# 0xk0ry/HTR-VT

Measured on AMD Instinct MI355X. Metric: line-images/sec (64x1024, global B=128, 128 per GPU) fwd+bwd+CTC, higher is better.
Workload: dtype bf16; 1 GPU; HTR-VT (d768/4L/6h, nb_cls 80) training step: fwd + fused CTC + bwd + AdamW; image=1x64x1024, batch_per_gpu=128, global_batch=128, mask=span 0.4/8 (run/iam.sh), parallelism=dp1, graph_replay=False

## Files before the change

htr-vt_amd/csrc/gemm_halo_impl.h:

```cpp
#pragma once
#include "gemm_dma_impl.h"

namespace {

template <int BN>
struct HaloGeo {
  static constexpr int BM = 256;
  static constexpr int A_PIECES = 40;
  static constexpr int A_STAGE = A_PIECES * 1024;
  static constexpr int B_STAGE = Geo<BN>::BYTES;
  static constexpr int NP_B = B_STAGE / 1024 / 4;
  static constexpr int NP_AH = A_PIECES / 2 / 4;
  static constexpr unsigned B_BASE = 2 * A_STAGE;
  static constexpr int LDS_BYTES = 2 * A_STAGE + 3 * B_STAGE;
  static_assert(B_STAGE % 4096 == 0, "B pieces divide over the four loader waves");
  static_assert(LDS_BYTES <= 160 * 1024, "LDS");
};


typedef float f32x4h_t __attribute__((ext_vector_type(4)));
template <int BN, int TM, int TN>
__device__ __forceinline__ void halo_mma16(f32x4h_t (&a4)[2 * TM][2 * TN], const char* sa, const char* sb, int shift, int wm, int wn,
                                           int lane) {
  const int arow16 = wm * 64 + (lane & 15), ag = lane >> 4;
// ... 40 lines not shown
  const int lr = lane & 15, lg = lane >> 4;
  float s1[2 * TN], s2[2 * TN];
#pragma unroll
  for (int j = 0; j < 2 * TN; ++j) s1[j] = s2[j] = 0.f;
  if (active) {
#pragma unroll
    for (int j = 0; j < 2 * TN; ++j) {
      const int n = n0 + wn * TN * 32 + 16 * j + lr;
      const bool nok = n < p.N;
#pragma unroll
      for (int i = 0; i < 2 * TM; ++i) {
#pragma unroll
        for (int r = 0; r < 4; ++r) {
          const int m = m0 + wm * 64 + 16 * i + 4 * lg + r;
          const float a = a4[i][j][r];
          if constexpr (CSTATS) {
            s1[j] += a;
            s2[j] = fmaf(a, a, s2[j]);
          }
          if (nok && m < p.M) {
            const long long o = (long long)m * p.ldc + n;
            float v = a * p.alpha;
            if (Rf != nullptr) v += Rf[o];
            Cf[o] = v;
          }
        }
      }
    }
  }
  if constexpr (CSTATS) {
    if (p.colstats != nullptr) {
      float* red = reinterpret_cast<float*>(smem);
#pragma unroll
      for (int j = 0; j < 2 * TN; ++j) {
        float a = s1[j], q = s2[j];
        a += __shfl_xor(a, 16, 64); q += __shfl_xor(q, 16, 64);
        a += __shfl_xor(a, 32, 64); q += __shfl_xor(q, 32, 64);
        if (lane < 16 && active) {
          const int c = wn * TN * 32 + 16 * j + lane;
          red[(wm * BN + c) * 2 + 0] = a;
          red[(wm * BN + c) * 2 + 1] = q;
        }
      }
      __syncthreads();
      for (int c = threadIdx.x; c < BN; c += NTH) {
        const int n = n0 + c;
        if (n < p.N) {
          float a = 0.f, q = 0.f;
#pragma unroll
          for (int w = 0; w < 4; ++w) {
            a += red[(w * BN + c) * 2];
            q += red[(w * BN + c) * 2 + 1];
          }
          float* dst = p.colstats + (long long)tile_m * 2 * p.N;
          dst[n] = a;
          dst[p.N + n] = q;
        }
      }
    }
  }
}

template <int BN, class P>
__device__ __forceinline__ void gemm_halo_s2_body(const P& p, const int block_x) {
  using H = HaloGeo<BN>;
  constexpr int BM = 256, NWC = 8, NW_TOTAL = 12, TM = 2, TN = BN / 64;
  extern __shared__ __attribute__((aligned(16))) char smem[];

  const int ntiles = p.tiles_m * p.tiles_n;
  int id = block_x;
  if ((ntiles & 7) == 0) id = (id & 7) * (ntiles >> 3) + (id >> 3);
  const int tile_m = id / p.tiles_n, tile_n = id - tile_m * p.tiles_n;
  const int n0 = tile_n * BN;
  const int sw = p.sw, ncls = 2 * sw;
  const int segs = p.Wq >> 8;
  const int per_row = ncls * segs;
  const int rowq = tile_m / per_row, rem = tile_m - rowq * per_row;
  const int cidx = rem / segs, seg = rem - cidx * segs;
  const int ca = 1 - cidx / sw;
  const int cb = sw == 2 ? 1 - (cidx & 1) : 0;
  const int bimg = rowq / p.Hq, hq = rowq - bimg * p.Hq;
  const int wq0 = seg << 8;
  const int Hh = p.Ho, Ww = p.Wo, Cs = p.Co;
  const int nrow = ca ? 2 : 1;
  const int dyp = ca ? (0 | (2 << 2)) : 1;
  const int dhp = ca ? (1 | (0 << 2)) : 0;
  const int ncol = sw == 1 ? 3 : (cb ? 2 : 1);
  const int dxp = sw == 1 ? (0 | (1 << 2) | (2 << 4)) : (cb ? (0 | (2 << 2)) : 1);
  const int shp = sw == 1 ? (2 | (1 << 2) | (0 << 4)) : (cb ? (2 | (1 << 2)) : 1);
  const int NC = p.Cpad / BK;
  const bool has_x = p.extra_off != 0 && ca == 0 && cb == 0;
  const int nmain = nrow * NC;
  const int ngroups = nmain + (has_x ? NC : 0);
  const int xtap = p.kh * p.kw;
  const int kend = (xtap + 1) * p.Cpad;

  const int lane = threadIdx.x & 63;
  const int wave = __builtin_amdgcn_readfirstlane(threadIdx.x >> 6);
  const bool consumer = wave < NWC;
  const int lw = (wave - NWC) & 3;
  const int wm = (wave >> 1) & 3, wn = wave & 1;
  if (!consumer) __builtin_amdgcn_s_setprio(3);

  DmaLoader<BN, HTRVT_KMAJOR, 0, 4> lb;
  lb.init(p, p.B, p.ldb, n0, p.N, lw, lane);
  const unsigned long long ba = (unsigned long long)p.A;
  const i32x4_t rsrcA = i32x4_t{(int)(unsigned)(ba & 0xffffffffull), (int)(unsigned)((ba >> 32) & 0xffffull), (int)OOB, 0x00020000};
  const int rho0 = lw * 8 + (lane >> 3);
  const int cgA = (lane & 7) ^ Geo<BM>::swz(rho0);
  const unsigned lane_off = (unsigned)((wq0 - 1 + rho0) * Cs + cgA * 8) * 2u;
  const unsigned lds0 = lds_addr_of(smem);

  unsigned abase0, abase1, abasex;
  {
    const int h0 = hq + (dhp & 3), h1 = hq + ((dhp >> 2) & 3);
    abase0 = (unsigned)h0 < (unsigned)Hh ? (unsigned)(((bimg * Hh + h0) * Ww) * Cs) * 2u : OOB;
    abase1 = (nrow > 1 && (unsigned)h1 < (unsigned)Hh) ? (unsigned)(((bimg * Hh + h1) * Ww) * Cs) * 2u : OOB;
    abasex = has_x ? (unsigned)(((bimg * Hh + hq) * Ww) * Cs) * 2u + p.extra_off : OOB;
  }
  const int nslot = nrow + (has_x ? 1 : 0);
  auto group_base = [](int as, int ac, int nslot_, int nrow_, unsigned b0, unsigned b1, unsigned bx) -> unsigned {
    const unsigned rb = as >= nslot_ ? OOB : (as == nrow_ ? bx : (as == 0 ? b0 : b1));
    return rb < OOB ? rb + (unsigned)(ac * BK) * 2u : OOB;
  };
  auto issueA = [&](int half, int ast, unsigned gbase, int ac) {
    const bool chok = gbase < OOB && ac * BK + cgA * 8 < Cs;
#pragma unroll
    for (int i = 0; i < H::NP_AH; ++i) {
      const int ii = half * H::NP_AH + i;
      const int rho = rho0 + 32 * ii;
      const int w = wq0 - 1 + rho;
      const bool v = chok && rho < 258 && (unsigned)w < (unsigned)Ww;
      const unsigned voff = v ? gbase + lane_off + (unsigned)(32 * ii * Cs) * 2u : OOB;
      dma16(rsrcA, __builtin_amdgcn_readfirstlane(lds0 + ast * H::A_STAGE + (lw + 4 * ii) * 1024), voff);
    }
  };
  int bs = 0, bc = 0, bj = 0;
  auto issueB = [&](int bst) {
    int k0 = kend;
    if (bs < nslot) {
      const bool x = bs == nrow;
      const int tap = x ? xtap : ((dyp >> (2 * bs)) & 3) * 3 + ((dxp >> (2 * bj)) & 3);
      k0 = tap * p.Cpad + bc * BK;
      if (++bj == (x ? 1 : ncol)) {
        bj = 0;
        if (++bc == NC) {
          bc = 0;
          ++bs;
        }
      }
    }
    lb.template issue<true>(p, lds0 + H::B_BASE + bst * H::B_STAGE, k0, kend, lw);
  };

  const int m0 = (bimg * p.Hi + 2 * hq + ca) * p.Wi + sw * wq0 + cb;

  if (consumer) {
    f32x4h_t a4[2 * TM][2 * TN];
#pragma unroll
    for (int i = 0; i < 2 * TM; ++i)
#pragma unroll
      for (int j = 0; j < 2 * TN; ++j) a4[i][j] = f32x4h_t{0.f, 0.f, 0.f, 0.f};
    __builtin_amdgcn_s_barrier();
    int bst = 0;
    for (int g = 0; g < ngroups; ++g) {
      const int n = g < nmain ? ncol : 1;
      const char* sa = smem + (g & 1) * H::A_STAGE;
      for (int j = 0; j < n; ++j) {
        const int shift = g < nmain ? (shp >> (2 * j)) & 3 : 1;
// ... 43 lines not shown
            asm volatile("s_waitcnt vmcnt(%0)" ::"n"(H::NP_B) : "memory");
          }
        } else {
          issueB(fill);
          if (!last) {
            issueA(j, nast, ngb, nc);
            asm volatile("s_waitcnt vmcnt(%0)" ::"n"(H::NP_B + H::NP_AH) : "memory");
          } else {
            asm volatile("s_waitcnt vmcnt(%0)" ::"n"(H::NP_B) : "memory");
          }
        }
        __builtin_amdgcn_s_barrier();
        bst = bst == 2 ? 0 : bst + 1;
      }
      gs = ns;
      gc = nc;
    }
    asm volatile("s_waitcnt vmcnt(0)" ::: "memory");
    __builtin_amdgcn_s_barrier();
    f32x16_t acc[TM][TN];
#pragma unroll
    for (int i = 0; i < TM; ++i)
#pragma unroll
      for (int j = 0; j < TN; ++j)
#pragma unroll
        for (int r = 0; r < 16; ++r) acc[i][j][r] = 0.f;
    epilogue_staged<TN, BN, BM, NW_TOTAL, true, false, P, 16>(acc, p, 0ll, m0, n0, wm, wn, tile_m, lane, wave, smem, false, sw);
  }
}

template <int BN>
__global__ __launch_bounds__(768) void gemm_halo_s2_kernel(const KParams p) {
  typedef const __attribute__((address_space(4))) KParams KP;
  (void)p;
  KP* kp = (KP*)__builtin_amdgcn_kernarg_segment_ptr();
  gemm_halo_s2_body<BN>(*kp, (int)blockIdx.x);
}

template <int BN>
int launch_halo_s2(const KParams& p, hipStream_t st) {
  constexpr int LDS = HaloGeo<BN>::LDS_BYTES;
  static bool attr_done = false;
  auto kern = gemm_halo_s2_kernel<BN>;
  if (!attr_done) {
    hipError_t e = hipFuncSetAttribute(reinterpret_cast<const void*>(kern), hipFuncAttributeMaxDynamicSharedMemorySize, LDS);
    if (e != hipSuccess) {
      set_error("hipFuncSetAttribute(%d B LDS): %s", LDS, hipGetErrorString(e));
      return -2;
    }
    attr_done = true;
  }
  hipLaunchKernelGGL(kern, dim3(p.tiles_m * p.tiles_n), dim3(768), LDS, st, p);
  set_last_kernel("gemm_halo_s2_kernel<%d>", BN);
  const int rc = check_launch("gemm_halo_s2_kernel");
  return rc ? rc : 1;
}

template <int BN>
struct HaloFs2Geo {
  static constexpr int NPO = 9, NPE = 8;
  static constexpr int X_BYTES = 4 * NPO * 1024, Y_BYTES = 4 * NPE * 1024;
  static constexpr int B_STAGE = Geo<BN>::BYTES;
  static constexpr int NP_B = B_STAGE / 1024 / 4;
  static constexpr unsigned Y_BASE = X_BYTES, B_BASE = X_BYTES + Y_BYTES;
  static constexpr int LDS_BYTES = X_BYTES + Y_BYTES + 3 * B_STAGE;
  static_assert(B_STAGE % 4096 == 0 && LDS_BYTES <= 160 * 1024, "LDS");
  static_assert(LDS_BYTES >= BN * Stg<256>::CST, "the staged epilogue's column-major image");
};

template <int BN, bool F32, class P>
__device__ __forceinline__ void gemm_halo_fs2_body(const P& p, const int block_x) {
  using H = HaloFs2Geo<BN>;
  constexpr int BM = 256, NWC = 8, NW_TOTAL = 12, TM = 2, TN = BN / 64;
  extern __shared__ __attribute__((aligned(16))) char smem[];

  const int ntiles = p.tiles_m * p.tiles_n;
  int id = block_x;
  if ((ntiles & 7) == 0) id = (id & 7) * (ntiles >> 3) + (id >> 3);
  const int tile_m = id / p.tiles_n, tile_n = id - tile_m * p.tiles_n;
  const int m0 = tile_m * BM, n0 = tile_n * BN;
  const int rowo = m0 / p.Wo, wo0 = m0 - rowo * p.Wo;
  const int bimg = rowo / p.Ho, ho = rowo - bimg * p.Ho;
  const int NC = p.Cpad / BK;
  const int NU = 3 * NC;

  const int lane = threadIdx.x & 63;
  const int wave = __builtin_amdgcn_readfirstlane(threadIdx.x >> 6);
  const int wm = (wave >> 1) & 3, wn = wave & 1;

  if (wave < NWC) {
    f32x4h_t a4[2 * TM][2 * TN];
#pragma unroll
    for (int i = 0; i < 2 * TM; ++i)
#pragma unroll
      for (int j = 0; j < 2 * TN; ++j) a4[i][j] = f32x4h_t{0.f, 0.f, 0.f, 0.f};
    __builtin_amdgcn_s_barrier();
    for (int u = 0; u < NU; ++u) {
      halo_mma16<BN, TM, TN>(a4, smem, smem + H::B_BASE + 0 * H::B_STAGE, 0, wm, wn, lane);
      __builtin_amdgcn_s_barrier();
      halo_mma16<BN, TM, TN>(a4, smem, smem + H::B_BASE + 1 * H::B_STAGE, 1, wm, wn, lane);
      __builtin_amdgcn_s_barrier();
      halo_mma16<BN, TM, TN>(a4, smem + H::Y_BASE, smem + H::B_BASE + 2 * H::B_STAGE, 0, wm, wn, lane);
      __builtin_amdgcn_s_barrier();
    }
    __builtin_amdgcn_s_barrier();
    if constexpr (F32) {
      halo_epilogue_f32<BN, TM, TN, NW_TOTAL * 64, true>(a4, p, m0, n0, wm, wn, tile_m, lane, smem, true);
    } else {
      f32x16_t acc[TM][TN];
      halo_acc16_to_32<TM, TN>(acc, a4);
      epilogue_staged<TN, BN, BM, NW_TOTAL, false, true, P, 16>(acc, p, 0ll, m0, n0, wm, wn, tile_m, lane, wave, smem, true);
    }
  } else {
    const int lw = (wave - NWC) & 3;
    __builtin_amdgcn_s_setprio(3);
    DmaLoader<BN, HTRVT_KMAJOR, 0, 4> lb;
    lb.init(p, p.B, p.ldb, n0, p.N, lw, lane);
    const unsigned long long ba = (unsigned long long)p.A;
    const i32x4_t rsrcA = i32x4_t{(int)(unsigned)(ba & 0xffffffffull), (int)(unsigned)((ba >> 32) & 0xffffull), (int)OOB, 0x00020000};
    const int Hh = p.Hi, Ww = p.Wi, Cs = p.Ci;
    const int rho0 = lw * 8 + (lane >> 3);
    const int cgA = (lane & 7) ^ Geo<BM>::swz(rho0);
    const int wsrc0 = 2 * (wo0 + rho0) - 1;
    const unsigned lane_off = (unsigned)(wsrc0 * Cs + cgA * 8) * 2u;
    const unsigned lds0 = lds_addr_of(smem);
    auto issueA = [&](int par, int udy, int ucc, bool uvalid) {
      const int hh = ho * p.sh + udy - 1;
      const bool rowok = uvalid && (unsigned)hh < (unsigned)Hh;
      const unsigned gbase = (unsigned)(((bimg * Hh + hh) * Ww + par) * Cs + ucc * BK) * 2u;
      const bool chok = ucc * BK + cgA * 8 < Cs;
      if (par == 0) {
#pragma unroll
        for (int i = 0; i < H::NPO; ++i) {
          const int rho = rho0 + 32 * i, w = wsrc0 + 64 * i;
          const bool v = rowok && chok && rho < 257 && (unsigned)w < (unsigned)Ww;
          dma16(rsrcA, __builtin_amdgcn_readfirstlane(lds0 + (lw + 4 * i) * 1024), v ? gbase + lane_off + (unsigned)(64 * i * Cs) * 2u : OOB);
        }
      } else {
#pragma unroll
        for (int i = 0; i < H::NPE; ++i) {
          const int w = wsrc0 + 1 + 64 * i;
          const bool v = rowok && chok && (unsigned)w < (unsigned)Ww;
          dma16(rsrcA, __builtin_amdgcn_readfirstlane(lds0 + H::Y_BASE + (lw + 4 * i) * 1024), v ? gbase + lane_off + (unsigned)(64 * i * Cs) * 2u : OOB);
        }
      }
    };
    auto issueB = [&](int bst, int udy, int ucc, int dx, bool uvalid) {
      lb.template issue<true>(p, lds0 + H::B_BASE + bst * H::B_STAGE, uvalid ? (udy * 3 + dx) * p.Cpad + ucc * BK : p.K, p.K, lw);
    };
    issueA(0, 0, 0, true);
    issueB(0, 0, 0, 0, true);
    issueB(1, 0, 0, 2, true);
    asm volatile("s_waitcnt vmcnt(%0)" ::"n"(H::NP_B) : "memory");
    __builtin_amdgcn_s_barrier();
    int udy = 0, ucc = 0;
    for (int u = 0; u < NU; ++u) {
      int ndy = udy, ncc = ucc + 1;
      if (ncc == NC) {
        ncc = 0;
        ++ndy;
      }
      const bool nvalid = u + 1 < NU;
      issueB(2, udy, ucc, 1, true);
      issueA(1, udy, ucc, true);
      asm volatile("s_waitcnt vmcnt(%0)" ::"n"(H::NP_B + H::NPE) : "memory");
      __builtin_amdgcn_s_barrier();
      issueB(0, ndy, ncc, 0, nvalid);
      asm volatile("s_waitcnt vmcnt(%0)" ::"n"(H::NP_B) : "memory");
      __builtin_amdgcn_s_barrier();
      issueA(0, ndy, ncc, nvalid);
      issueB(1, ndy, ncc, 2, nvalid);
      asm volatile("s_waitcnt vmcnt(%0)" ::"n"(H::NP_B) : "memory");
      __builtin_amdgcn_s_barrier();
      udy = ndy;
      ucc = ncc;
    }
    asm volatile("s_waitcnt vmcnt(0)" ::: "memory");
    __builtin_amdgcn_s_barrier();
    if constexpr (F32) {
      f32x4h_t z4[2 * TM][2 * TN];
#pragma unroll
      for (int i = 0; i < 2 * TM; ++i)
#pragma unroll
        for (int j = 0; j < 2 * TN; ++j) z4[i][j] = f32x4h_t{0.f, 0.f, 0.f, 0.f};
      halo_epilogue_f32<BN, TM, TN, NW_TOTAL * 64, true>(z4, p, m0, n0, wm, wn, tile_m, lane, smem, false);
    } else {
    f32x16_t acc[TM][TN];
#pragma unroll
    for (int i = 0; i < TM; ++i)
#pragma unroll
      for (int j = 0; j < TN; ++j)
#pragma unroll
        for (int r = 0; r < 16; ++r) acc[i][j][r] = 0.f;
    epilogue_staged<TN, BN, BM, NW_TOTAL, false, true, P, 16>(acc, p, 0ll, m0, n0, wm, wn, tile_m, lane, wave, smem, false);
    }
  }
}

template <int BN, bool F32 = false>
__global__ __launch_bounds__(768) void gemm_halo_fs2_kernel(const KParams p) {
  typedef const __attribute__((address_space(4))) KParams KP;
  (void)p;
  KP* kp = (KP*)__builtin_amdgcn_kernarg_segment_ptr();
  gemm_halo_fs2_body<BN, F32>(*kp, (int)blockIdx.x);
}

template <int BN, bool F32 = false>
int launch_halo_fs2(const KParams& p, hipStream_t st) {
  constexpr int LDS = HaloFs2Geo<BN>::LDS_BYTES;
  static bool attr_done = false;
  auto kern = gemm_halo_fs2_kernel<BN, F32>;
  if (!attr_done) {
    hipError_t e = hipFuncSetAttribute(reinterpret_cast<const void*>(kern), hipFuncAttributeMaxDynamicSharedMemorySize, LDS);
    if (e != hipSuccess) {
      set_error("hipFuncSetAttribute(%d B LDS): %s", LDS, hipGetErrorString(e));
      return -2;
    }
    attr_done = true;
  }
  hipLaunchKernelGGL(kern, dim3(p.tiles_m * p.tiles_n), dim3(768), LDS, st, p);
  if (F32) set_last_kernel("gemm_halo_fs2_kernel<%d, f32>", BN);
  else set_last_kernel("gemm_halo_fs2_kernel<%d>", BN);
  const int rc = check_launch("gemm_halo_fs2_kernel");
  return rc ? rc : 1;
}

template <int BN, bool DGRAD, bool F32, class P>
__device__ __forceinline__ void gemm_halo_body(const P& p, const int block_x) {
  using H = HaloGeo<BN>;
  constexpr int BM = 256, NWC = 8, NW_TOTAL = 12, TM = 2, TN = BN / 64;
  extern __shared__ __attribute__((aligned(16))) char smem[];

  const int ntiles = p.tiles_m * p.tiles_n;
  int id = block_x;
  if ((ntiles & 7) == 0) id = (id & 7) * (ntiles >> 3) + (id >> 3);
  const int tile_m = id / p.tiles_n, tile_n = id - tile_m * p.tiles_n;
  const int m0 = tile_m * BM, n0 = tile_n * BN;
  const int Hh = DGRAD ? p.Ho : p.Hi, Ww = DGRAD ? p.Wo : p.Wi, Cs = DGRAD ? p.Co : p.Ci;
  const int rowi = m0 / Ww, w0 = m0 - rowi * Ww;
  const int Hm = DGRAD ? Hh : p.Ho;
  const int bimg = rowi / Hm, hrow = rowi - bimg * Hm;
  const int NC = p.Cpad / BK;
  const int NG = 3 * NC;

  const int lane = threadIdx.x & 63;
  const int wave = __builtin_amdgcn_readfirstlane(threadIdx.x >> 6);
  const int wm = (wave >> 1) & 3, wn = wave & 1;

  if (wave < NWC) {
    f32x4h_t a4[2 * TM][2 * TN];
#pragma unroll
    for (int i = 0; i < 2 * TM; ++i)
#pragma unroll
      for (int j = 0; j < 2 * TN; ++j) a4[i][j] = f32x4h_t{0.f, 0.f, 0.f, 0.f};
    __builtin_amdgcn_s_barrier();
    for (int g = 0; g < NG; ++g) {
      const char* sa = smem + (g & 1) * H::A_STAGE;
      halo_mma16<BN, TM, TN>(a4, sa, smem + H::B_BASE + 0 * H::B_STAGE, DGRAD ? 2 : 0, wm, wn, lane);
      __builtin_amdgcn_s_barrier();
      halo_mma16<BN, TM, TN>(a4, sa, smem + H::B_BASE + 1 * H::B_STAGE, 1, wm, wn, lane);
      __builtin_amdgcn_s_barrier();
      halo_mma16<BN, TM, TN>(a4, sa, smem + H::B_BASE + 2 * H::B_STAGE, DGRAD ? 0 : 2, wm, wn, lane);
      __builtin_amdgcn_s_barrier();
    }
    __builtin_amdgcn_s_barrier();
    if constexpr (F32) {
      halo_epilogue_f32<BN, TM, TN, NW_TOTAL * 64, !DGRAD>(a4, p, m0, n0, wm, wn, tile_m, lane, smem, true);
    } else {
      f32x16_t acc[TM][TN];
      halo_acc16_to_32<TM, TN>(acc, a4);
      epilogue_staged<TN, BN, BM, NW_TOTAL, DGRAD, !DGRAD, P, 16>(acc, p, 0ll, m0, n0, wm, wn, tile_m, lane, wave, smem, true);
    }
  } else {
    const int lw = (wave - NWC) & 3;
    __builtin_amdgcn_s_setprio(3);
    DmaLoader<BN, HTRVT_KMAJOR, 0, 4> lb;
    lb.init(p, p.B, p.ldb, n0, p.N, lw, lane);
    const unsigned long long ba = (unsigned long long)p.A;
    const i32x4_t rsrcA = i32x4_t{(int)(unsigned)(ba & 0xffffffffull), (int)(unsigned)((ba >> 32) & 0xffffull), (int)OOB, 0x00020000};
    const int rho0 = lw * 8 + (lane >> 3);
    const int cgA = (lane & 7) ^ Geo<BM>::swz(rho0);
    const unsigned lane_off = (unsigned)((w0 - 1 + rho0) * Cs + cgA * 8) * 2u;
    const unsigned lds0 = lds_addr_of(smem);
    auto issueA = [&](int half, int ast, int gdy, int gcc) {
      const int hh = DGRAD ? hrow + 1 - gdy : hrow * p.sh + gdy - 1;
      const bool rowok = (unsigned)hh < (unsigned)Hh;
      const unsigned gbase = (unsigned)(((bimg * Hh + hh) * Ww) * Cs + gcc * BK) * 2u;
      const bool chok = gcc * BK + cgA * 8 < Cs;
#pragma unroll
      for (int i = 0; i < H::NP_AH; ++i) {
        const int ii = half * H::NP_AH + i;
        const int rho = rho0 + 32 * ii;
        const int w = w0 - 1 + rho;
        const bool v = rowok && chok && rho < 258 && (unsigned)w < (unsigned)Ww;
        const unsigned voff = v ? gbase + lane_off + (unsigned)(32 * ii * Cs) * 2u : OOB;
        dma16(rsrcA, __builtin_amdgcn_readfirstlane(lds0 + ast * H::A_STAGE + (lw + 4 * ii) * 1024), voff);
      }
    };
    auto issueB = [&](int bst, int gdy, int gcc, int dx) {
      lb.template issue<true>(p, lds0 + H::B_BASE + bst * H::B_STAGE, (gdy * 3 + dx) * p.Cpad + gcc * BK, p.K, lw);
    };
    issueA(0, 0, 0, 0);
    issueA(1, 0, 0, 0);
    issueB(0, 0, 0, 0);
    issueB(1, 0, 0, 1);
    asm volatile("s_waitcnt vmcnt(%0)" ::"n"(H::NP_B) : "memory");
    __builtin_amdgcn_s_barrier();
    int gdy = 0, gcc = 0;
    for (int g = 0; g < NG - 1; ++g) {
      int ndy = gdy, ncc = gcc + 1;
      if (ncc == NC) {
        ncc = 0;
        ++ndy;
      }
      const int nast = (g + 1) & 1;
      issueB(2, gdy, gcc, 2);
      issueA(0, nast, ndy, ncc);
      asm volatile("s_waitcnt vmcnt(%0)" ::"n"(H::NP_B + H::NP_AH) : "memory");
      __builtin_amdgcn_s_barrier();
      issueB(0, ndy, ncc, 0);
      issueA(1, nast, ndy, ncc);
      asm volatile("s_waitcnt vmcnt(%0)" ::"n"(H::NP_B + H::NP_AH) : "memory");
      __builtin_amdgcn_s_barrier();
      issueB(1, ndy, ncc, 1);
      asm volatile("s_waitcnt vmcnt(%0)" ::"n"(H::NP_B) : "memory");
      __builtin_amdgcn_s_barrier();
      gdy = ndy;
      gcc = ncc;
    }
    issueB(2, gdy, gcc, 2);
    asm volatile("s_waitcnt vmcnt(%0)" ::"n"(H::NP_B) : "memory");
    __builtin_amdgcn_s_barrier();
    asm volatile("s_waitcnt vmcnt(0)" ::: "memory");
    __builtin_amdgcn_s_barrier();
    __builtin_amdgcn_s_barrier();
    __builtin_amdgcn_s_barrier();
    if constexpr (F32) {
      f32x4h_t z4[2 * TM][2 * TN];
#pragma unroll
      for (int i = 0; i < 2 * TM; ++i)
#pragma unroll
        for (int j = 0; j < 2 * TN; ++j) z4[i][j] = f32x4h_t{0.f, 0.f, 0.f, 0.f};
      halo_epilogue_f32<BN, TM, TN, NW_TOTAL * 64, !DGRAD>(z4, p, m0, n0, wm, wn, tile_m, lane, smem, false);
    } else {
    f32x16_t acc[TM][TN];
#pragma unroll
    for (int i = 0; i < TM; ++i)
#pragma unroll
      for (int j = 0; j < TN; ++j)
#pragma unroll
        for (int r = 0; r < 16; ++r) acc[i][j][r] = 0.f;
    epilogue_staged<TN, BN, BM, NW_TOTAL, DGRAD, !DGRAD, P, 16>(acc, p, 0ll, m0, n0, wm, wn, tile_m, lane, wave, smem, false);
    }
  }
}

template <int BN, bool DGRAD, bool F32 = false>
__global__ __launch_bounds__(768) void gemm_halo_kernel(const KParams p) {
  typedef const __attribute__((address_space(4))) KParams KP;
  (void)p;
  KP* kp = (KP*)__builtin_amdgcn_kernarg_segment_ptr();
  gemm_halo_body<BN, DGRAD, F32>(*kp, (int)blockIdx.x);
}

template <int BN, bool DGRAD, bool F32 = false>
int launch_halo(const KParams& p, hipStream_t st) {
  using H = HaloGeo<BN>;
  static bool attr_done = false;
  auto kern = gemm_halo_kernel<BN, DGRAD, F32>;
  if (!attr_done) {
    hipError_t e = hipFuncSetAttribute(reinterpret_cast<const void*>(kern), hipFuncAttributeMaxDynamicSharedMemorySize, H::LDS_BYTES);
    if (e != hipSuccess) {
      set_error("hipFuncSetAttribute(%d B LDS): %s", H::LDS_BYTES, hipGetErrorString(e));
      return -2;
    }
    attr_done = true;
  }
  hipLaunchKernelGGL(kern, dim3(p.tiles_m * p.tiles_n), dim3(768), H::LDS_BYTES, st, p);
  if (F32) set_last_kernel("gemm_halo_kernel<%d, %s, f32>", BN, DGRAD ? "true" : "false");
  else set_last_kernel("gemm_halo_kernel<%d, %s>", BN, DGRAD ? "true" : "false");
  const int rc = check_launch("gemm_halo_kernel");
  return rc ? rc : 1;
}

}
```

htr-vt_amd/csrc/gemm_hwgrad_impl.h:

```cpp
#pragma once
#include "gemm_dma_impl.h"

namespace {

template <int CC, int BN>
struct HwGeo {
  static constexpr int NW = 12, NTH = NW * 64;
  static constexpr int BM = 3 * CC;
  static constexpr int XROWB = CC * 2, XCPR = CC / 8;
  static constexpr int XRPP = 1024 / XROWB;
  static constexpr int XPIECES = (66 + XRPP - 1) / XRPP;
  static constexpr int XBYTES = XPIECES * 1024;
  static constexpr int YBYTES = Geo<BN, NW>::BYTES, YPIECES = YBYTES / 1024;
  static constexpr int STAGE = XBYTES + YBYTES;
  static constexpr int NSTAGE = 3;
  static constexpr int LDS_BYTES = NSTAGE * STAGE;
  static constexpr int TM = CC / 64, TN = BN / 64;
  static constexpr int WROWS = CC / 2;
  static_assert(CC == 64 || CC == 128, "channel chunk");
  static constexpr int NWY = YPIECES % NW == 0 ? NW : 8;
  static_assert(YPIECES % NWY == 0, "dY pieces divide over the issuing waves");
  static constexpr int NPY = YPIECES / NWY;
  static constexpr int NPX_MAX = (XPIECES + NW - 1) / NW;
  static_assert(LDS_BYTES <= 160 * 1024, "LDS");
  static __device__ __forceinline__ int xrot(int r) { return CC == 128 ? 4 * (r & 3) : 4 * ((r >> 1) & 1); }
};

template <int CC, int BN, bool PAIR, class P>
__device__ __forceinline__ void gemm_hwgrad_body(const P& p, const int block_x) {
  using H = HwGeo<CC, BN>;
  using T = bf16_t;
  constexpr int TM = H::TM, TN = H::TN, NW = H::NW;
  static_assert(!PAIR || CC == 128, "paired units are 64 channels wide");
  extern __shared__ __attribute__((aligned(16))) char smem[];

  const int NCC = PAIR ? p.Cpad / 64 : p.Cpad / CC;
  const int nunits = 3 * NCC;
  const int tiles_m = PAIR ? (nunits + 1) / 2 : nunits;
  const int ntiles = tiles_m * p.tiles_n;
  int id = block_x, z = blockIdx.z;
  if (p.split_k > 1 && (p.split_k & 7) == 0) {
    const int chunk = block_x / (8 * ntiles), r = block_x - chunk * 8 * ntiles;
    z = chunk * 8 + (r & 7);
    id = r >> 3;
  } else if (p.split_k > 1 && gridDim.z == 1) {
    xcd_range_map(block_x, (int)gridDim.x, ntiles, z, id);
  }
  const int tm = id / p.tiles_n, tile_n = id - tm * p.tiles_n;
  int dyu[2], ciu[2];
  bool uok[2];
#pragma unroll
  for (int u = 0; u < 2; ++u) {
    const int t = PAIR ? 2 * tm + u : tm;
    uok[u] = t < nunits;
    const int tt = uok[u] ? t : 0;
    dyu[u] = tt / NCC;
    ciu[u] = (tt - dyu[u] * NCC) * (PAIR ? 64 : CC);
  }
  const int n0 = tile_n * BN;
  int kbeg = 0, kend = p.K;
  long long coff = 0;
  if (p.split_k > 1) {
    kbeg = z * p.kchunk;
    kend = min(p.K, kbeg + p.kchunk);
    coff = (long long)z * p.slab_stride;
  }

  const int lane = threadIdx.x & 63;
  const int wave = __builtin_amdgcn_readfirstlane(threadIdx.x >> 6);
  const int wm = wave >> 1, wn = wave & 1;
  const int dx = wm / (CC / 64 * 1 + (CC == 64 ? 1 : 0));
  const int crow = (wm & 1) * H::WROWS;

  DmaLoader<BN, HTRVT_MNMAJOR, 0, H::NWY> ly;
  const bool yload = wave < H::NWY;
  ly.init(p, p.B, p.ldb, n0, p.N, yload ? wave : 0, lane);
  const unsigned long long xa = (unsigned long long)p.A;
  const i32x4_t rsrcX = i32x4_t{(int)(unsigned)(xa & 0xffffffffull), (int)(unsigned)((xa >> 32) & 0xffffull), (int)OOB, 0x00020000};
  const int npx = (wave < H::XPIECES - NW * (H::NPX_MAX - 1)) ? H::NPX_MAX : H::NPX_MAX - 1;
  const int per_tile = npx + (wave < H::NWY ? H::NPY : 0);
  auto wait_one_tile_in_flight = [&]() {
    switch (per_tile) {
      case 0: asm volatile("s_waitcnt vmcnt(0)" ::: "memory"); break;
      case 1: asm volatile("s_waitcnt vmcnt(1)" ::: "memory"); break;
      case 2: asm volatile("s_waitcnt vmcnt(2)" ::: "memory"); break;
      case 3: asm volatile("s_waitcnt vmcnt(3)" ::: "memory"); break;
      case 4: asm volatile("s_waitcnt vmcnt(4)" ::: "memory"); break;
      default: asm volatile("s_waitcnt vmcnt(5)" ::: "memory"); break;
    }
  };
  static_assert(H::NPX_MAX + H::NPY <= 5, "vmcnt switch");
  const unsigned lds0 = lds_addr_of(smem);
  const int Hh = p.Hi, Ww = p.Wi;
  int iq_row = kbeg / Ww, iq_w0 = kbeg - iq_row * Ww, iq_k = kbeg;
  auto issue = [&](int stage) {
    const unsigned sbase = lds0 + stage * H::STAGE;
    const int bimg = iq_row / p.Ho, hrow = iq_row - bimg * p.Ho;
    bool rowok[2];
    unsigned gbase[2];
#pragma unroll
    for (int u = 0; u < (PAIR ? 2 : 1); ++u) {
      const int hh = hrow * p.sh + dyu[u] - 1;
      rowok[u] = uok[u] && iq_k < kend && (unsigned)hh < (unsigned)Hh;
      gbase[u] = (unsigned)(((bimg * Hh + hh) * Ww + iq_w0 - 1) * p.Ci + ciu[u]) * 2u;
    }
#pragma unroll
    for (int i = 0; i < H::NPX_MAX; ++i) {
      if (i < npx) {
        const int pi = wave + NW * i;
        const int r = pi * H::XRPP + lane / H::XCPR;
        const int cd = lane % H::XCPR;
        int cs = cd - H::xrot(r);
        cs += cs < 0 ? H::XCPR : 0;
        const int w = iq_w0 - 1 + r;
        const int u = PAIR ? cs >> 3 : 0;
        const int cu = PAIR ? cs & 7 : cs;
        const bool ro = PAIR ? (u ? rowok[1] : rowok[0]) : rowok[0];
        const int ci = PAIR ? (u ? ciu[1] : ciu[0]) : ciu[0];
        const unsigned gb = PAIR ? (u ? gbase[1] : gbase[0]) : gbase[0];
        const bool v = ro && r < 66 && (unsigned)w < (unsigned)Ww && ci + cu * 8 < p.Ci;
        const unsigned voff = v ? gb + (unsigned)(r * p.Ci + cu * 8) * 2u : OOB;
        dma16(rsrcX, __builtin_amdgcn_readfirstlane(sbase + pi * 1024), voff);
      }
    }
    if (yload) ly.template issue<false>(p, sbase + H::XBYTES, iq_k, kend, wave);
    iq_k += BK;
    iq_w0 += BK;
    if (iq_w0 >= Ww) {
      iq_w0 = 0;
      ++iq_row;
    }
  };

  f32x16_t acc[TM][TN];
#pragma unroll
  for (int i = 0; i < TM; ++i)
#pragma unroll
    for (int j = 0; j < TN; ++j)
#pragma unroll
      for (int r = 0; r < 16; ++r) acc[i][j][r] = 0.f;

  const int nkt = (kend - kbeg + BK - 1) / BK;
  issue(0);
  issue(1);
  wait_one_tile_in_flight();
  __builtin_amdgcn_s_barrier();

  const int g = lane >> 4, q = (lane & 15) >> 2, pp = lane & 3, hq = g >> 1;
  auto xfrag = [&](const char* xs, int i, int s) {
    const int r0 = 16 * s + 8 * hq + q + dx;
    const int cb = (crow + 32 * i) / 8 + 2 * (g & 1) + (pp >> 1);
    int c0 = cb + H::xrot(r0), c1 = cb + H::xrot(r0 + 4);
    c0 -= c0 >= H::XCPR ? H::XCPR : 0;
    c1 -= c1 >= H::XCPR ? H::XCPR : 0;
    typedef __attribute__((address_space(3))) s16x4_t* lptr;
    const s16x4_t a = __builtin_amdgcn_ds_read_tr16_b64_v4i16((lptr)(xs + r0 * H::XROWB + c0 * 16 + (pp & 1) * 8));
    const s16x4_t b = __builtin_amdgcn_ds_read_tr16_b64_v4i16((lptr)(xs + (r0 + 4) * H::XROWB + c1 * 16 + (pp & 1) * 8));
    const s16x8_t r = {a.x, a.y, a.z, a.w, b.x, b.y, b.z, b.w};
    return __builtin_bit_cast(bf16x8_t, r);
  };

  auto kstep_load = [&](const char* xs, const char* ys, int s, bf16x8_t (&fa)[TM], bf16x8_t (&fb)[TN]) {
#pragma unroll
    for (int i = 0; i < TM; ++i) fa[i] = xfrag(xs, i, s);
#pragma unroll
    for (int j = 0; j < TN; ++j) fb[j] = frag_read<BN, HTRVT_MNMAJOR>(ys, wn * TN + j, s, lane);
  };
  auto kstep_mma = [&](const bf16x8_t (&fa)[TM], const bf16x8_t (&fb)[TN]) {
#pragma unroll
    for (int i = 0; i < TM; ++i)
#pragma unroll
      for (int j = 0; j < TN; ++j)
        acc[i][j] = __builtin_amdgcn_mfma_f32_32x32x16_bf16(fa[i], fb[j], acc[i][j], 0, 0, 0);
  };
  auto kstep = [&](const char* xs, const char* ys, int s) {
    bf16x8_t fa[TM], fb[TN];
    kstep_load(xs, ys, s, fa, fb);
    kstep_mma(fa, fb);
  };
  bf16x8_t fa2[TM], fb2[TN];
  if (nkt > 0) {
    kstep(smem, smem + H::XBYTES, 0);
    kstep(smem, smem + H::XBYTES, 1);
    kstep_load(smem, smem + H::XBYTES, 2, fa2, fb2);
  }
  int cur = 0, nxt = 2;
  for (int kt = 0; kt < nkt; ++kt) {
    const char* xs = smem + cur * H::STAGE;
    const char* ys = xs + H::XBYTES;
    asm volatile("s_waitcnt vmcnt(0)" ::: "memory");
    __builtin_amdgcn_s_barrier();
    issue(nxt);
    kstep_mma(fa2, fb2);
    kstep(xs, ys, 3);
    cur = cur == 2 ? 0 : cur + 1;
    nxt = nxt == 2 ? 0 : nxt + 1;
    if (kt + 1 < nkt) {
      const char* xn = smem + cur * H::STAGE;
      const char* yn = xn + H::XBYTES;
      kstep(xn, yn, 0);
      kstep(xn, yn, 1);
      kstep_load(xn, yn, 2, fa2, fb2);
    }
  }
  asm volatile("s_waitcnt vmcnt(0)" ::: "memory");

  const int un = PAIR ? (wm & 1) : 0;
  const int mrow0 = (dyu[un] * 3 + dx) * p.Cpad + ciu[un] + (PAIR ? 0 : crow);
  gemm_epilogue<T, TM, TN, 1, BN, H::NTH, false>(acc, p, p.C, coff, mrow0, n0 + wn * TN * 32, 0, n0, 0, lane, smem, uok[un]);
}

template <int CC, int BN, int SW = 1>
struct Hw16Geo {
  static constexpr int NW = 12, NTH = NW * 64;
  static constexpr int XROWB = CC * 2, XCPR = CC / 8;
  static constexpr int EVEN0 = 80;
  static constexpr int XROWS = SW == 1 ? 66 : EVEN0 + 64;
  static constexpr int XPIECES = (XROWS * XROWB + 1023) / 1024;
  static constexpr int XBYTES = XPIECES * 1024;
  static constexpr int YROWB = BN * 2, YCPR = BN / 8;
  static constexpr int YBYTES = 64 * YROWB, YPIECES = YBYTES / 1024;
  static constexpr int STAGE = XBYTES + YBYTES, NSTAGE = 3, LDS_BYTES = NSTAGE * STAGE;
  static constexpr int RT = CC / 32, CT = BN / 32;
  static constexpr int NPX = (XPIECES + NW - 1) / NW, NPY = YPIECES / NW;
  static_assert(CC == 96 && BN == 192 && (SW == 1 || SW == 2) && YPIECES % NW == 0 && LDS_BYTES <= 160 * 1024, "geometry");
  static constexpr bool HOLD = CC == 96;
  static __device__ __forceinline__ int xrot(int r) { return CC == 96 ? 2 * ((r >> 3) & 1) : 4 * (r & 3) + 2 * ((r >> 3) & 1); }
  static __device__ __forceinline__ int yrot(int k) { return BN == 192 ? 4 * ((k >> 1) & 1) + 2 * ((k >> 3) & 1) : 4 * (k & 3) + 2 * ((k >> 3) & 1); }
};

typedef float f32x4w_t __attribute__((ext_vector_type(4)));

template <int CC, int BN, int SW, class P>
__device__ __forceinline__ void gemm_hwgrad16_body(const P& p, const int block_x) {
  using H = Hw16Geo<CC, BN, SW>;
  constexpr int NW = H::NW, RT = H::RT, CT = H::CT;
  extern __shared__ __attribute__((aligned(16))) char smem[];

  const int NCC = p.Cpad / CC;
  const int nunits = 3 * NCC;
  const int ntiles = nunits * p.tiles_n;
  int id = block_x, z = blockIdx.z;
  if (p.split_k > 1 && (p.split_k & 7) == 0) {
    const int chunk = block_x / (8 * ntiles), r = block_x - chunk * 8 * ntiles;
    z = chunk * 8 + (r & 7);
    id = r >> 3;
  } else if (p.split_k > 1 && gridDim.z == 1) {
    xcd_range_map(block_x, (int)gridDim.x, ntiles, z, id);
  }
  const int tm = id / p.tiles_n, tile_n = id - tm * p.tiles_n;
  const int dyu = tm / NCC, ciu = (tm - dyu * NCC) * CC;
  const int n0 = tile_n * BN;
  int kbeg = 0, kend = p.K;
  long long coff = 0;
  if (p.split_k > 1) {
    kbeg = z * p.kchunk;
    kend = min(p.K, kbeg + p.kchunk);
    coff = (long long)z * p.slab_stride;
  }

  const int lane = threadIdx.x & 63;
  const int wave = __builtin_amdgcn_readfirstlane(threadIdx.x >> 6);
  const int wm = wave >> 1, wn = wave & 1;
  const int dx = wm >> 1;
  const int crow = (wm & 1) * (CC / 2);

  const unsigned long long xa = (unsigned long long)p.A, ya = (unsigned long long)p.B;
  const i32x4_t rsrcX = i32x4_t{(int)(unsigned)(xa & 0xffffffffull), (int)(unsigned)((xa >> 32) & 0xffffull), (int)OOB, 0x00020000};
  const i32x4_t rsrcY = i32x4_t{(int)(unsigned)(ya & 0xffffffffull), (int)(unsigned)((ya >> 32) & 0xffffull), (int)OOB, 0x00020000};
  int xr[H::NPX], xc[H::NPX];
  bool xok[H::NPX];
#pragma unroll
  for (int i = 0; i < H::NPX; ++i) {
    const int pi = wave + NW * i;
    const int q = pi * 1024 + lane * 16;
    const int r = q / H::XROWB, cd = (q - r * H::XROWB) >> 4;
    int cs = cd - H::xrot(r);
    cs += cs < 0 ? H::XCPR : 0;
    xr[i] = SW == 1 ? r : (r < H::EVEN0 ? 2 * r - 1 : 2 * (r - H::EVEN0));
    xc[i] = cs;
    xok[i] = pi < H::XPIECES && (SW == 1 ? r < 66 : (r < 65 || (r >= H::EVEN0 && r < H::EVEN0 + 64))) && ciu + cs * 8 < p.Ci;
  }
  unsigned yoff[H::NPY];
  int ykr[H::NPY];
#pragma unroll
  for (int i = 0; i < H::NPY; ++i) {
    const int sidx = (wave + NW * i) * 64 + lane;
    const int kr = sidx / H::YCPR, cl = sidx - kr * H::YCPR;
    int cg = cl - H::yrot(kr);
    cg += cg < 0 ? H::YCPR : 0;
    const int col = n0 + cg * 8;
    ykr[i] = kr;
    yoff[i] = col < p.N ? (unsigned)kr * (unsigned)(p.ldb * 2) + (unsigned)col * 2u : OOB;
  }
  const unsigned lds0 = lds_addr_of(smem);
  const int Hh = p.Hi, Ww = p.Wi, Wk = p.Wo;
  int iq_row = kbeg / Wk, iq_w0 = kbeg - iq_row * Wk, iq_k = kbeg;
  auto issue = [&](int stage) {
    const unsigned sbase = lds0 + stage * H::STAGE;
    const int bimg = iq_row / p.Ho, hrow = iq_row - bimg * p.Ho;
    const int hh = hrow * p.sh + dyu - 1;
    const bool rowok = iq_k < kend && (unsigned)hh < (unsigned)Hh;
    const int wfirst = SW == 1 ? iq_w0 - 1 : 2 * iq_w0;
    const unsigned gbase = (unsigned)(((bimg * Hh + hh) * Ww + wfirst) * p.Ci + ciu) * 2u;
#pragma unroll
    for (int i = 0; i < H::NPX; ++i) {
      if (wave + NW * i < H::XPIECES) {
        const int w = wfirst + xr[i];
        const bool v = rowok && xok[i] && (unsigned)w < (unsigned)Ww;
        const unsigned voff = v ? gbase + (unsigned)(xr[i] * p.Ci + xc[i] * 8) * 2u : OOB;
        dma16(rsrcX, __builtin_amdgcn_readfirstlane(sbase + (wave + NW * i) * 1024), voff);
      }
    }
    const unsigned ybase = (unsigned)iq_k * (unsigned)(p.ldb * 2);
#pragma unroll
    for (int i = 0; i < H::NPY; ++i) {
      const bool v = yoff[i] < OOB && iq_k + ykr[i] < kend;
      dma16(rsrcY, __builtin_amdgcn_readfirstlane(sbase + H::XBYTES + (wave + NW * i) * 1024), v ? ybase + yoff[i] : OOB);
    }
    iq_k += BK;
    iq_w0 += BK;
    if (iq_w0 >= Wk) {
      iq_w0 = 0;
      ++iq_row;
    }
  };

  f32x4w_t acc[RT][CT];
#pragma unroll
  for (int i = 0; i < RT; ++i)
#pragma unroll
    for (int j = 0; j < CT; ++j) acc[i][j] = f32x4w_t{0.f, 0.f, 0.f, 0.f};

  const int nkt = (kend - kbeg + BK - 1) / BK;
  issue(0);
  issue(1);
  if (wave + NW * (H::NPX - 1) < H::XPIECES) asm volatile("s_waitcnt vmcnt(%0)" ::"n"(H::NPX + H::NPY) : "memory");
  else asm volatile("s_waitcnt vmcnt(%0)" ::"n"(H::NPX - 1 + H::NPY) : "memory");
  __builtin_amdgcn_s_barrier();

  const int g = lane >> 4, q = (lane & 15) >> 2, pp = lane & 3;
  typedef __attribute__((address_space(3))) s16x4_t* lptr;
  auto xfrag = [&](const char* xs, int i, int s) {
    const int r0 = 32 * s + 8 * g + q + (SW == 1 ? dx : (dx == 1 ? H::EVEN0 : (dx >> 1)));
    const int cb = (crow + 16 * i) / 8 + (pp >> 1);
    int c0 = cb + H::xrot(r0), c1 = cb + H::xrot(r0 + 4);
    c0 -= c0 >= H::XCPR ? H::XCPR : 0;
    c1 -= c1 >= H::XCPR ? H::XCPR : 0;
    const s16x4_t a = __builtin_amdgcn_ds_read_tr16_b64_v4i16((lptr)(xs + r0 * H::XROWB + c0 * 16 + (pp & 1) * 8));
    const s16x4_t b = __builtin_amdgcn_ds_read_tr16_b64_v4i16((lptr)(xs + (r0 + 4) * H::XROWB + c1 * 16 + (pp & 1) * 8));
    const s16x8_t r = {a.x, a.y, a.z, a.w, b.x, b.y, b.z, b.w};
    return __builtin_bit_cast(bf16x8_t, r);
  };
  auto yfrag = [&](const char* ys, int j, int s) {
    const int k0 = 32 * s + 8 * g + q;
    const int cb = (wn * (BN / 2) + 16 * j) / 8 + (pp >> 1);
    int c0 = cb + H::yrot(k0), c1 = cb + H::yrot(k0 + 4);
    c0 -= c0 >= H::YCPR ? H::YCPR : 0;
    c1 -= c1 >= H::YCPR ? H::YCPR : 0;
    const s16x4_t a = __builtin_amdgcn_ds_read_tr16_b64_v4i16((lptr)(ys + k0 * H::YROWB + c0 * 16 + (pp & 1) * 8));
    const s16x4_t b = __builtin_amdgcn_ds_read_tr16_b64_v4i16((lptr)(ys + (k0 + 4) * H::YROWB + c1 * 16 + (pp & 1) * 8));
    const s16x8_t r = {a.x, a.y, a.z, a.w, b.x, b.y, b.z, b.w};
    return __builtin_bit_cast(bf16x8_t, r);
  };
  auto kstep_load = [&](const char* xs, const char* ys, int s, bf16x8_t (&fa)[RT], bf16x8_t (&fb)[CT]) {
#pragma unroll
    for (int i = 0; i < RT; ++i) fa[i] = xfrag(xs, i, s);
#pragma unroll
    for (int j = 0; j < CT; ++j) fb[j] = yfrag(ys, j, s);
  };
  auto kstep_mma = [&](const bf16x8_t (&fa)[RT], const bf16x8_t (&fb)[CT]) {
#pragma unroll
    for (int i = 0; i < RT; ++i)
#pragma unroll
      for (int j = 0; j < CT; ++j) acc[i][j] = __builtin_amdgcn_mfma_f32_16x16x32_bf16(fa[i], fb[j], acc[i][j], 0, 0, 0);
  };
  if constexpr (H::HOLD) {
  bf16x8_t fa2[RT], fb2[CT];
  if (nkt > 0) {
    bf16x8_t fa[RT], fb[CT];
    kstep_load(smem, smem + H::XBYTES, 0, fa, fb);
    kstep_mma(fa, fb);
    kstep_load(smem, smem + H::XBYTES, 1, fa2, fb2);
  }
  int cur = 0, nxt = 2;
  for (int kt = 0; kt < nkt; ++kt) {
    asm volatile("s_waitcnt vmcnt(0)" ::: "memory");
    __builtin_amdgcn_s_barrier();
    issue(nxt);
    kstep_mma(fa2, fb2);
    cur = cur == 2 ? 0 : cur + 1;
    nxt = nxt == 2 ? 0 : nxt + 1;
    if (kt + 1 < nkt) {
      const char* xn = smem + cur * H::STAGE;
      const char* yn = xn + H::XBYTES;
      bf16x8_t fa[RT], fb[CT];
      kstep_load(xn, yn, 0, fa, fb);
      kstep_mma(fa, fb);
      kstep_load(xn, yn, 1, fa2, fb2);
    }
  }
  } else {
  int cur = 0, nxt = 2;
  for (int kt = 0; kt < nkt; ++kt) {
    const char* xs = smem + cur * H::STAGE;
    const char* ys = xs + H::XBYTES;
    if (kt > 0) {
      asm volatile("s_waitcnt vmcnt(0)" ::: "memory");
      __builtin_amdgcn_s_barrier();
    }
    issue(nxt);
#pragma unroll
    for (int s2 = 0; s2 < 2; ++s2) {
      bf16x8_t fa[RT], fb[CT];
      kstep_load(xs, ys, s2, fa, fb);
      kstep_mma(fa, fb);
    }
// ... 88 lines not shown
```

Measured before the change: 4030 line-images/s.

## Skip zero-padding kernel rows in halo conv GEMMs and weight-grad kernels

The halo conv GEMM kernels (fprop, dgrad, fs2 and the subpixel variant) now compute how many of the three kernel-height taps fall inside the image and loop only over those, instead of always running all three and loading zeros for the padded rows. The weight-grad kernels count only the K-tiles whose input rows are live, and skip dead rows in the loader. They also reorder split-K tile assignment so the tiles with the most live work start first, which should balance the load. This adds per-block control logic and risks mismatched pipeline counts at image borders.

```diff
diff --git a/htr-vt_amd/csrc/gemm_halo_impl.h b/htr-vt_amd/csrc/gemm_halo_impl.h
--- a/htr-vt_amd/csrc/gemm_halo_impl.h
+++ b/htr-vt_amd/csrc/gemm_halo_impl.h
@@ -146,9 +146,10 @@
   const int bimg = rowq / p.Hq, hq = rowq - bimg * p.Hq;
   const int wq0 = seg << 8;
   const int Hh = p.Ho, Ww = p.Wo, Cs = p.Co;
-  const int nrow = ca ? 2 : 1;
-  const int dyp = ca ? (0 | (2 << 2)) : 1;
-  const int dhp = ca ? (1 | (0 << 2)) : 0;
+  const bool two = ca && hq + 1 < Hh;
+  const int nrow = two ? 2 : 1;
+  const int dyp = two ? (0 | (2 << 2)) : (ca ? 2 : 1);
+  const int dhp = two ? (1 | (0 << 2)) : 0;
   const int ncol = sw == 1 ? 3 : (cb ? 2 : 1);
   const int dxp = sw == 1 ? (0 | (1 << 2) | (2 << 4)) : (cb ? (0 | (2 << 2)) : 1);
   const int shp = sw == 1 ? (2 | (1 << 2) | (0 << 4)) : (cb ? (2 | (1 << 2)) : 1);
@@ -358,7 +359,9 @@
   const int rowo = m0 / p.Wo, wo0 = m0 - rowo * p.Wo;
   const int bimg = rowo / p.Ho, ho = rowo - bimg * p.Ho;
   const int NC = p.Cpad / BK;
-  const int NU = 3 * NC;
+  const int ulo = __builtin_amdgcn_readfirstlane((unsigned)(ho * p.sh - 1) < (unsigned)p.Hi ? 0 : 1);
+  const int uhi = __builtin_amdgcn_readfirstlane((unsigned)(ho * p.sh + 1) < (unsigned)p.Hi ? 2 : 1);
+  const int NU = (uhi - ulo + 1) * NC;
 
   const int lane = threadIdx.x & 63;
   const int wave = __builtin_amdgcn_readfirstlane(threadIdx.x >> 6);
@@ -424,12 +427,12 @@
     auto issueB = [&](int bst, int udy, int ucc, int dx, bool uvalid) {
       lb.template issue<true>(p, lds0 + H::B_BASE + bst * H::B_STAGE, uvalid ? (udy * 3 + dx) * p.Cpad + ucc * BK : p.K, p.K, lw);
     };
-    issueA(0, 0, 0, true);
-    issueB(0, 0, 0, 0, true);
-    issueB(1, 0, 0, 2, true);
+    issueA(0, ulo, 0, true);
+    issueB(0, ulo, 0, 0, true);
+    issueB(1, ulo, 0, 2, true);
     asm volatile("s_waitcnt vmcnt(%0)" ::"n"(H::NP_B) : "memory");
     __builtin_amdgcn_s_barrier();
-    int udy = 0, ucc = 0;
+    int udy = ulo, ucc = 0;
     for (int u = 0; u < NU; ++u) {
       int ndy = udy, ncc = ucc + 1;
       if (ncc == NC) {
@@ -517,7 +520,10 @@
   const int Hm = DGRAD ? Hh : p.Ho;
   const int bimg = rowi / Hm, hrow = rowi - bimg * Hm;
   const int NC = p.Cpad / BK;
-  const int NG = 3 * NC;
+  const int hh0 = DGRAD ? hrow + 1 : hrow * p.sh - 1, hh2 = DGRAD ? hrow - 1 : hrow * p.sh + 1;
+  const int glo = __builtin_amdgcn_readfirstlane((unsigned)hh0 < (unsigned)Hh ? 0 : 1);
+  const int ghi = __builtin_amdgcn_readfirstlane((unsigned)hh2 < (unsigned)Hh ? 2 : 1);
+  const int NG = (ghi - glo + 1) * NC;
 
   const int lane = threadIdx.x & 63;
   const int wave = __builtin_amdgcn_readfirstlane(threadIdx.x >> 6);
@@ -576,13 +582,13 @@
     auto issueB = [&](int bst, int gdy, int gcc, int dx) {
       lb.template issue<true>(p, lds0 + H::B_BASE + bst * H::B_STAGE, (gdy * 3 + dx) * p.Cpad + gcc * BK, p.K, lw);
     };
-    issueA(0, 0, 0, 0);
-    issueA(1, 0, 0, 0);
-    issueB(0, 0, 0, 0);
-    issueB(1, 0, 0, 1);
+    issueA(0, 0, glo, 0);
+    issueA(1, 0, glo, 0);
+    issueB(0, glo, 0, 0);
+    issueB(1, glo, 0, 1);
     asm volatile("s_waitcnt vmcnt(%0)" ::"n"(H::NP_B) : "memory");
     __builtin_amdgcn_s_barrier();
-    int gdy = 0, gcc = 0;
+    int gdy = glo, gcc = 0;
     for (int g = 0; g < NG - 1; ++g) {
       int ndy = gdy, ncc = gcc + 1;
       if (ncc == NC) {
diff --git a/htr-vt_amd/csrc/gemm_hwgrad_impl.h b/htr-vt_amd/csrc/gemm_hwgrad_impl.h
--- a/htr-vt_amd/csrc/gemm_hwgrad_impl.h
+++ b/htr-vt_amd/csrc/gemm_hwgrad_impl.h
@@ -26,6 +26,45 @@
   static __device__ __forceinline__ int xrot(int r) { return CC == 128 ? 4 * (r & 3) : 4 * ((r >> 1) & 1); }
 };
 
+template <class F>
+__device__ __forceinline__ int hw_live_ktiles(int kbeg, int kend, int w0, int h, int Wk, int Ho, F live) {
+  int n = 0;
+  for (int k = kbeg; k < kend;) {
+    const int px = min(Wk - w0, kend - k);
+    if (live(h)) n += (px + BK - 1) / BK;
+    k += px;
+    w0 = 0;
+    h = h + 1 == Ho ? 0 : h + 1;
+  }
+  return n;
+}
+
+__device__ __forceinline__ int hw_long_first_tile(int s, int ntiles) {
+  const int T = ntiles / 3;
+  return s < T ? s + T : (s < 2 * T ? s - T : s);
+}
+__device__ __forceinline__ void hw_xcd_range_map_long_first(int b, int total, int ntiles, int& z, int& id) {
+  const int x = b & 7, s = b >> 3;
+  const int q = total >> 3, r = total & 7;
+  const int P = x * q + (x < r ? x : r), n = q + (x < r ? 1 : 0);
+  const int T = ntiles / 3;
+  auto nlong = [&](int a) {
+    const int za = a / ntiles, m = a - za * ntiles;
+    return za * T + min(max(m - T, 0), T);
+  };
+  const int l0 = nlong(P), nl = nlong(P + n) - l0;
+  if (s < nl) {
+    const int k = l0 + s;
+    z = k / T;
+    id = T + (k - z * T);
+  } else {
+    const int k = P - l0 + s - nl;
+    z = k / (2 * T);
+    const int m = k - z * 2 * T;
+    id = m < T ? m : m + T;
+  }
+}
+
 template <int CC, int BN, bool PAIR, class P>
 __device__ __forceinline__ void gemm_hwgrad_body(const P& p, const int block_x) {
   using H = HwGeo<CC, BN>;
@@ -42,9 +81,10 @@
   if (p.split_k > 1 && (p.split_k & 7) == 0) {
     const int chunk = block_x / (8 * ntiles), r = block_x - chunk * 8 * ntiles;
     z = chunk * 8 + (r & 7);
-    id = r >> 3;
+    id = PAIR ? r >> 3 : hw_long_first_tile(r >> 3, ntiles);
   } else if (p.split_k > 1 && gridDim.z == 1) {
-    xcd_range_map(block_x, (int)gridDim.x, ntiles, z, id);
+    if (PAIR) xcd_range_map(block_x, (int)gridDim.x, ntiles, z, id);
+    else hw_xcd_range_map_long_first(block_x, (int)gridDim.x, ntiles, z, id);
   }
   const int tm = id / p.tiles_n, tile_n = id - tm * p.tiles_n;
   int dyu[2], ciu[2];
@@ -93,9 +133,25 @@
   const unsigned lds0 = lds_addr_of(smem);
   const int Hh = p.Hi, Ww = p.Wi;
   int iq_row = kbeg / Ww, iq_w0 = kbeg - iq_row * Ww, iq_k = kbeg;
+  int iq_h = iq_row % p.Ho;
+  auto row_live = [&](int h) {
+    bool live = (unsigned)(h * p.sh + dyu[0] - 1) < (unsigned)Hh;
+    if (PAIR) live = live || (uok[1] && (unsigned)(h * p.sh + dyu[1] - 1) < (unsigned)Hh);
+    return live;
+  };
+  const int nkt = hw_live_ktiles(kbeg, kend, iq_w0, iq_h, Ww, p.Ho, row_live);
+  auto skip_dead_rows = [&]() {
+    while (iq_k < kend && !row_live(iq_h)) {
+      iq_k += Ww - iq_w0;
+      iq_w0 = 0;
+      ++iq_row;
+      iq_h = iq_h + 1 == p.Ho ? 0 : iq_h + 1;
+    }
+  };
+  skip_dead_rows();
   auto issue = [&](int stage) {
     const unsigned sbase = lds0 + stage * H::STAGE;
-    const int bimg = iq_row / p.Ho, hrow = iq_row - bimg * p.Ho;
+    const int bimg = iq_row / p.Ho, hrow = iq_h;
     bool rowok[2];
     unsigned gbase[2];
 #pragma unroll
@@ -129,6 +185,8 @@
     if (iq_w0 >= Ww) {
       iq_w0 = 0;
       ++iq_row;
+      iq_h = iq_h + 1 == p.Ho ? 0 : iq_h + 1;
+      skip_dead_rows();
     }
   };
 
@@ -140,7 +198,6 @@
 #pragma unroll
       for (int r = 0; r < 16; ++r) acc[i][j][r] = 0.f;
 
-  const int nkt = (kend - kbeg + BK - 1) / BK;
   issue(0);
   issue(1);
   wait_one_tile_in_flight();
@@ -244,9 +301,9 @@
   if (p.split_k > 1 && (p.split_k & 7) == 0) {
     const int chunk = block_x / (8 * ntiles), r = block_x - chunk * 8 * ntiles;
     z = chunk * 8 + (r & 7);
-    id = r >> 3;
+    id = hw_long_first_tile(r >> 3, ntiles);
   } else if (p.split_k > 1 && gridDim.z == 1) {
-    xcd_range_map(block_x, (int)gridDim.x, ntiles, z, id);
+    hw_xcd_range_map_long_first(block_x, (int)gridDim.x, ntiles, z, id);
   }
   const int tm = id / p.tiles_n, tile_n = id - tm * p.tiles_n;
   const int dyu = tm / NCC, ciu = (tm - dyu * NCC) * CC;
@@ -296,9 +353,21 @@
   const unsigned lds0 = lds_addr_of(smem);
   const int Hh = p.Hi, Ww = p.Wi, Wk = p.Wo;
   int iq_row = kbeg / Wk, iq_w0 = kbeg - iq_row * Wk, iq_k = kbeg;
+  int iq_h = iq_row % p.Ho;
+  auto row_live = [&](int h) { return (unsigned)(h * p.sh + dyu - 1) < (unsigned)Hh; };
+  const int nkt = hw_live_ktiles(kbeg, kend, iq_w0, iq_h, Wk, p.Ho, row_live);
+  auto skip_dead_rows = [&]() {
+    while (iq_k < kend && !row_live(iq_h)) {
+      iq_k += Wk - iq_w0;
+      iq_w0 = 0;
+      ++iq_row;
+      iq_h = iq_h + 1 == p.Ho ? 0 : iq_h + 1;
+    }
+  };
+  skip_dead_rows();
   auto issue = [&](int stage) {
     const unsigned sbase = lds0 + stage * H::STAGE;
-    const int bimg = iq_row / p.Ho, hrow = iq_row - bimg * p.Ho;
+    const int bimg = iq_row / p.Ho, hrow = iq_h;
     const int hh = hrow * p.sh + dyu - 1;
     const bool rowok = iq_k < kend && (unsigned)hh < (unsigned)Hh;
     const int wfirst = SW == 1 ? iq_w0 - 1 : 2 * iq_w0;
@@ -323,6 +392,8 @@
     if (iq_w0 >= Wk) {
       iq_w0 = 0;
       ++iq_row;
+      iq_h = iq_h + 1 == p.Ho ? 0 : iq_h + 1;
+      skip_dead_rows();
     }
   };
 
@@ -332,7 +403,6 @@
 #pragma unroll
     for (int j = 0; j < CT; ++j) acc[i][j] = f32x4w_t{0.f, 0.f, 0.f, 0.f};
 
-  const int nkt = (kend - kbeg + BK - 1) / BK;
   issue(0);
   issue(1);
   if (wave + NW * (H::NPX - 1) < H::XPIECES) asm volatile("s_waitcnt vmcnt(%0)" ::"n"(H::NPX + H::NPY) : "memory");
```

New measurement: 4265 line-images/s (median of 6 runs). 5.8% higher.
